# williamedwards/autompc

Hardware: AMD Instinct MI355X
Metric: MPC solves/sec (MPPI, n_samples x horizon rollouts + update per solve) (higher is better)
Workload: dtype f64; 1 GPU; c3: HalfCheetah (17-dim state, 6-dim ctrl), MLP 2x256, MPPI 4096 samples x 30 horizon; random-weight model, QuadCost Q=I R=0.01I F=I, sigma=1 lmda=1, 1 independent solve(s) per step per GPU, noise=device; n_samples=4096, horizon=30, state_dim=17, ctrl_dim=6, parallelism=independent solves per GPU (dp1)

## Files before the change

autompc_amd/csrc/mlp_tile.hpp:

```cpp
#pragma once
#include <hip/hip_runtime.h>

#include <type_traits>

#include "probe.hpp"

namespace ampc {

constexpr int kMaxHidden = 4;
constexpr int kMaxWaves = 8;

typedef double d4 __attribute__((ext_vector_type(4)));
typedef float f4 __attribute__((ext_vector_type(4)));

template <typename T> struct Acc;
template <> struct Acc<double> { using type = d4; };
template <> struct Acc<float> { using type = f4; };

__device__ __forceinline__ d4 mfma16(double a, double b, d4 c) {
  if constexpr (Probe::no_mfma) { c[0] += a * b; return c; }
  else return __builtin_amdgcn_mfma_f64_16x16x4f64(a, b, c, 0, 0, 0);
}
__device__ __forceinline__ f4 mfma16(float a, float b, f4 c) {
  if constexpr (Probe::no_mfma) { c[0] += a * b; return c; }
// ... 306 lines not shown
        b[nt] = __builtin_bit_cast(T, __builtin_amdgcn_raw_buffer_load_b64(r, vo + nt * 8u, sb, 0));
      else
        b[nt] = __builtin_bit_cast(T, __builtin_amdgcn_raw_buffer_load_b32(r, vo + nt * 4u, sb, 0));
    }
  }
}

template <typename T, int NT, int G>
__device__ __forceinline__ void load_group(rsrc_t r, unsigned so, unsigned lo, int g, T (&b)[G][NT]) {
#pragma unroll
  for (int kk = 0; kk < G; ++kk) load_frag<T, NT>(r, so + (unsigned)(g * G + kk) * 64u * NT, lo, b[kk]);
}

struct NoSide { __device__ __forceinline__ void operator()() const {} };
struct NoGroups {};

template <typename T, int NT, int MT, int KS, int G, bool PIPE = false, bool OWN = false, int SG = G,
          bool APERM = false, bool SWAP = false, typename Mid = NoSide, typename Groups = NoGroups,
          typename OwnFrag = NoGroups>
__device__ __forceinline__ void layer_mma_static(const T* __restrict__ A, int a_stride,
                                                 rsrc_t wr, unsigned wl, int lane,
                                                 const T (&first)[G][NT],
                                                 typename Acc<T>::type (&acc)[MT][NT], int rot = 0,
                                                 Mid&& mid = Mid(), Groups&& group_at = Groups(),
                                                 OwnFrag&& own_at = OwnFrag()) {
  static_assert(KS % G == 0 && G % SG == 0, "group sizes must divide the k extent");
  constexpr int NG = KS / G;
  constexpr int NS = KS / SG;
  constexpr int FS = G / SG;
  static_assert(!OWN || (NG & (NG - 1)) == 0, "rotated k order needs a power-of-two group count");
  const int i = lane & 15, q = lane >> 4;
  constexpr bool PINNED = !std::is_same<typename std::decay<Groups>::type, NoGroups>::value;
  constexpr bool REG0 = !std::is_same<typename std::decay<OwnFrag>::type, NoGroups>::value;
  static_assert(!REG0 || (OWN && MT == 1), "register fragments: the wave's own group of a 16-row tile");
  const T* arow = A + (APERM ? act_row<T>(i) : i) * a_stride + q;
  auto sub_group = [&](int g, int sub) {
    if constexpr (PINNED) return group_at(g) + 4 * SG * sub;
    else return (OWN ? arow + 4 * G * ((g + rot) & (NG - 1)) : arow + 4 * G * g) + 4 * SG * sub;
  };
  T b[2][SG][NT];
  if constexpr (FS == 1) {
#pragma unroll
    for (int kk = 0; kk < SG; ++kk)
#pragma unroll
      for (int nt = 0; nt < NT; ++nt) b[0][kk][nt] = first[kk][nt];
  }
#pragma unroll
  for (int sgi = 0; sgi < NS; ++sgi) {
    if (sgi + 1 >= FS && sgi + 1 < NS) load_group<T, NT, SG>(wr, wl, (unsigned)lane * NT, sgi + 1, b[(sgi + 1) & 1]);
    const int g = sgi / FS;
    const auto ag = sub_group(g, sgi % FS);
#pragma unroll
    for (int kk = 0; kk < SG; ++kk) {
      T a[MT];
#pragma unroll
      for (int mt = 0; mt < MT; ++mt) {
        if constexpr (REG0) a[mt] = sgi < FS ? own_at(sgi * SG + kk) : ag[4 * kk];
        else a[mt] = ag[mt * 16 * a_stride + 4 * kk];
      }
#pragma unroll
      for (int mt = 0; mt < MT; ++mt)
#pragma unroll
        for (int nt = 0; nt < NT; ++nt) {
          const T bv = (FS > 1 && sgi < FS) ? first[sgi * SG + kk][nt] : b[sgi & 1][kk][nt];
          constexpr bool REAL = KS < 16 ? kRealL0 : kRealHid;
          acc[mt][nt] = SWAP ? mfma16_x<REAL>(bv, a[mt], acc[mt][nt]) : mfma16_x<REAL>(a[mt], bv, acc[mt][nt]);
        }
    }
    if constexpr (PIPE && KS >= 8 && !Probe::no_sched) {
      if constexpr (Probe::vmem_first) {
        __builtin_amdgcn_sched_group_barrier(0x020, SG, 0);
        __builtin_amdgcn_sched_group_barrier(0x100, 2 * MT, 0);
#pragma unroll
        for (int i = 0; i < SG / 2; ++i) {
          __builtin_amdgcn_sched_group_barrier(0x008, 2 * MT * NT, 0);
          __builtin_amdgcn_sched_group_barrier(0x100, MT, 0);
        }
      } else if constexpr (sizeof(T) == 4 && (Probe::f32_ahead > 0 || Probe::f32_fine > 0)) {
        constexpr int AH = Probe::f32_ahead > 0 ? Probe::f32_ahead : 2;
        __builtin_amdgcn_sched_group_barrier(0x100, AH * MT, 0);
        if constexpr (Probe::f32_fine == 1) {
#pragma unroll
          for (int i = 0; i < SG; ++i) {
            __builtin_amdgcn_sched_group_barrier(0x008, MT * NT, 0);
            if (i + AH < SG) __builtin_amdgcn_sched_group_barrier(0x100, MT, 0);
            __builtin_amdgcn_sched_group_barrier(0x020, 1, 0);
          }
        } else if constexpr (Probe::f32_fine == 2) {
          constexpr int H1 = (MT * NT + 1) / 2, H2 = MT * NT - H1;
#pragma unroll
          for (int i = 0; i < SG; ++i) {
            __builtin_amdgcn_sched_group_barrier(0x008, H1, 0);
            if (i + AH < SG) __builtin_amdgcn_sched_group_barrier(0x100, MT, 0);
            if (H2 > 0) __builtin_amdgcn_sched_group_barrier(0x008, H2, 0);
            __builtin_amdgcn_sched_group_barrier(0x020, 1, 0);
          }
        } else if constexpr (Probe::f32_fine == 3) {
#pragma unroll
          for (int i = 0; i < SG; ++i) {
            __builtin_amdgcn_sched_group_barrier(0x008, MT * NT, 0);
            __builtin_amdgcn_sched_group_barrier(0x020, 1, 0);
            if (i + AH < SG) __builtin_amdgcn_sched_group_barrier(0x100, MT, 0);
          }
        } else {
#pragma unroll
          for (int i = 0; i < SG / 2; ++i) {
            __builtin_amdgcn_sched_group_barrier(0x008, 2 * MT * NT, 0);
            if (2 * i + AH < SG) __builtin_amdgcn_sched_group_barrier(0x100, MT, 0);
            if (2 * i + AH + 1 < SG) __builtin_amdgcn_sched_group_barrier(0x100, MT, 0);
            __builtin_amdgcn_sched_group_barrier(0x020, 2, 0);
          }
        }
      } else if (REG0 && sgi < FS) {
#pragma unroll
        for (int i = 0; i < SG / 2; ++i) {
          __builtin_amdgcn_sched_group_barrier(0x008, 2 * MT * NT, 0);
          __builtin_amdgcn_sched_group_barrier(0x020, 2, 0);
        }
      } else {
        __builtin_amdgcn_sched_group_barrier(0x100, 2 * MT, 0);
#pragma unroll
        for (int i = 0; i < SG / 2; ++i) {
          __builtin_amdgcn_sched_group_barrier(0x008, 2 * MT * NT, 0);
          __builtin_amdgcn_sched_group_barrier(0x100, MT, 0);
          __builtin_amdgcn_sched_group_barrier(0x020, 2, 0);
        }
      }
    }
    if (OWN && sgi == FS - 1) {
      lds_barrier();
      mid();
    }
    if constexpr (Probe::valu_pad) {
      if (KS >= 16 && sgi >= 2 && sgi < 10) {
        int padv = lane;
#pragma unroll
        for (int pi = 0; pi < 8; ++pi) asm volatile("v_add_u32 %0, %0, 1" : "+v"(padv));
        asm volatile("" :: "v"(padv));
      }
    }
    if constexpr (Probe::valu_pad64) {
      if (KS >= 16 && sgi >= 2 && sgi < 10) {
        double padd = (double)lane;
#pragma unroll
        for (int pi = 0; pi < 8; ++pi) asm volatile("v_add_f64 %0, %0, 1.0" : "+v"(padd));
        asm volatile("" :: "v"(padd));
      }
    }
  }
}


template <typename T, int NT, int MT, int W, bool DERIV = false, int LEAN = 0, typename SH = DynShape,
          bool WIDE = false, bool PINNED = false>
struct TileNet {
  using acc_t = typename Acc<T>::type;
  static constexpr int M = 16 * MT;
  static constexpr int HP = 16 * NT * W;
  static constexpr int KSH = HP / 4;
  static constexpr int KSW = KSH / W;
  static constexpr int KS0MAX = 12;
  static constexpr int GH = 8;
  static constexpr int NOMAX = WIDE ? 4 : 2;
  static constexpr bool OWN = (16 * NT == 4 * GH) && (((KSH / GH) & (KSH / GH - 1)) == 0);
  static constexpr bool PIN = PINNED && SH::kStatic && sizeof(T) == 8;
  static constexpr bool CHAIN = PIN && MT == 1 && !DERIV && !WIDE && LEAN == 0;
  static constexpr int BR = (CHAIN && W == 8) ? 4 : 1;
  static constexpr bool CHAIN_BIAS_LDS = CHAIN && BR == 1;

  static constexpr int KS0RES = sizeof(T) == 4 ? KS0MAX : 6;
  T pf0[KS0RES][NT];
  __device__ __forceinline__ static bool resident0(const MlpDev<T>& m) {
    return !Probe::no_res0 && LEAN < 2 && (sizeof(T) == 4 || MT == 1) && m.k1p <= 4 * KS0RES;
  }

  __device__ __forceinline__ static unsigned slice0(const MlpDev<T>& m, int w) {
    return (unsigned)(m.W(0) - m.WB()) + (unsigned)w * (unsigned)(m.k1p / 4) * 64u * NT;
  }
  __device__ __forceinline__ static unsigned slice_h(const MlpDev<T>& m, int l, int w) {
    return (unsigned)(m.W(l) - m.WB()) + (unsigned)w * (unsigned)KSH * 64u * NT;
  }
  rsrc_t wr;
  template <int KS> __device__ __forceinline__ const T (&first0() const)[KS][NT] {
    return reinterpret_cast<const T(&)[KS][NT]>(pf0);
  }
  template <int KS> __device__ __forceinline__ T (&first0())[KS][NT] {
    return reinterpret_cast<T(&)[KS][NT]>(pf0);
  }

  static constexpr bool RESIDENT_OUT = WIDE || (LEAN < 2 && !(MT == 4 && sizeof(T) == 8));
  T wout[KSW][NOMAX];

  __device__ __forceinline__ static void load_out(const MlpDev<T>& m, int w, int lane,
                                                  T (&dst)[KSW][NOMAX]) {
    if constexpr (WIDE) {
      const int tiles = m.nxp / 16;
      const T* wl = m.W(m.n_hidden) + ((size_t)w * KSW * 64 + lane) * tiles;
#pragma unroll
      for (int ks = 0; ks < KSW; ++ks)
#pragma unroll
        for (int n = 0; n < NOMAX; ++n) dst[ks][n] = n < tiles ? wl[(size_t)ks * 64 * tiles + n] : T(0);
    } else if (m.nxp == 16) {
      const T* wl = m.W(m.n_hidden) + ((size_t)w * KSW * 64 + lane);
#pragma unroll
      for (int ks = 0; ks < KSW; ++ks) { dst[ks][0] = wl[ks * 64]; dst[ks][1] = T(0); }
    } else {
      const T* wl = m.W(m.n_hidden) + ((size_t)w * KSW * 64 + lane) * 2;
#pragma unroll
      for (int ks = 0; ks < KSW; ++ks) { const vec_t<T, 2> v = *reinterpret_cast<const vec_t<T, 2>*>(wl + ks * 128); dst[ks][0] = v[0]; dst[ks][1] = v[1]; }
      if (m.tail4) {
        const T* wt = m.WT() + ((size_t)w * KSW * 64 + lane);
#pragma unroll
        for (int ks = 0; ks < KSW; ++ks) dst[ks][1] = wt[ks * 64];
      }
    }
  }

  static constexpr bool RESIDENT_BIAS = LEAN < 1 && (MT == 1);
  static constexpr int kResBias = 2;
  T bias_r[kResBias][NT][BR];
  T pfn[GH][NT];
  ProbeWave<Probe::wave_time> probe;

  lds_ptr<const T> bq_;
  static constexpr int RS = sizeof(T) == 8 ? 4 : 1;
  static constexpr int NGH = KSH / GH;
  lds_ptr<T> ep_[2][4];
  lds_ptr<const T> rd_[2][NGH];
  lds_ptr<const T> ro_;
  lds_ptr<const T> x0_;
  lds_ptr<T> pp_, pt_;
  int w_;

  __device__ __forceinline__ void pin(const MlpDev<T>& m_in, const TileLds& L_in, T* lds) {
    if constexpr (PIN) {
      const MlpDev<T> m = SH::template fold<T>(m_in);
      const TileLds L = SH::template fold_lds<T, M, W>(L_in);
      const int lane = threadIdx.x & 63;
      const int w = w_ = __builtin_amdgcn_readfirstlane(threadIdx.x >> 6);
      const int i = lane & 15, q = lane >> 4;
      const int as = L.act_stride;
      const bool pingpong = L.act2 != L.act;
#pragma unroll
      for (int b = 0; b < 2; ++b) {
        T* buf = lds + (b ? L.act2 : L.act);
        const bool read = b == 0 ? m.n_hidden > 1 : (pingpong && m.n_hidden > 2);
        const bool written = CHAIN ? read : (b == 0 || pingpong);
#pragma unroll
        for (int r = 0; r < 4; ++r) {
          if constexpr (CHAIN)
            ep_[b][r] = (written && r == 0) ? lds_pin(buf + i * as + 16 * NT * w + q) : lds_ptr<T>(nullptr);
          else
            ep_[b][r] = written ? lds_pin(buf + (act_row<T>(acc_row<T>(q, 0)) + RS * r) * as + 16 * NT * w + i) : ep_[0][r];
        }
#pragma unroll
        for (int g = 0; g < NGH; ++g) {
          const T* grp = buf + act_row<T>(i) * as + q + 4 * GH * (OWN ? ((g + w) & (NGH - 1)) : g);
          const bool used = OWN ? (g > 0 || !CHAIN) : g == 0;
          rd_[b][g] = (read && used) ? lds_pin(grp) : lds_ptr<const T>(nullptr);
        }
      }
      const T* last = lds + ((pingpong && ((m.n_hidden - 1) & 1)) ? L.act2 : L.act);
      ro_ = CHAIN ? lds_ptr<const T>(nullptr) : lds_pin(last + act_row<T>(i) * as + q + 4 * w * KSW);
      bq_ = (CHAIN && (CHAIN_BIAS_LDS || m.n_hidden > kResBias)) ? lds_pin(static_cast<const T*>(lds + L.bias + 16 * NT * w + q))
                                             : lds_ptr<const T>(nullptr);
      x0_ = lds_pin(static_cast<const T*>(lds + L.xu + i * L.xu_stride + q));
      const int ps = part_stride((int)sizeof(T), m.nxp);
      T* part = lds + L.part + w * M * ps;
      pp_ = lds_pin(part + acc_row<T>(q, 0) * ps + i);
      pt_ = m.tail4 ? lds_pin(part + tail_row(lane) * ps + 16 + tail_col(lane)) : pp_;
    }
  }

  __device__ __forceinline__ void init(const MlpDev<T>& m_in) {
    const MlpDev<T> m = SH::template fold<T>(m_in);
    const int lane = threadIdx.x & 63;
    const int w = __builtin_amdgcn_readfirstlane(threadIdx.x >> 6);
#pragma unroll
    for (int l = 0; l < kResBias; ++l)
#pragma unroll
      for (int nt = 0; nt < NT; ++nt)
#pragma unroll
        for (int r = 0; r < BR; ++r) {
          const int col = CHAIN ? 4 * r + (lane >> 4) : (lane & 15);
          bias_r[l][nt][r] = (RESIDENT_BIAS && !CHAIN_BIAS_LDS && l < m.n_hidden) ? m.B(l)[16 * (NT * w + nt) + col] : T(0);
        }
    wr = weight_rsrc(m.WB());
    if constexpr (RESIDENT_OUT) load_out(m, w, lane, wout);
    load0_all(m);
    if (m.n_hidden > 1) load_group<T, NT, GH>(wr, slice_h(m, 1, w), (unsigned)lane * NT, 0, pfn);
  }

  __device__ __forceinline__ void load0_all(const MlpDev<T>& m_in) {
    const MlpDev<T> m = SH::template fold<T>(m_in);
    const int lane = threadIdx.x & 63;
    const int w = __builtin_amdgcn_readfirstlane(threadIdx.x >> 6);
    const unsigned wl = slice0(m, w);
    const int ks0 = resident0(m) ? m.k1p / 4 : 2;
#pragma unroll
    for (int ks = 0; ks < KS0RES; ++ks) {
      T tmp[NT];
#pragma unroll
      for (int nt = 0; nt < NT; ++nt) tmp[nt] = T(0);
      if (ks < ks0) load_frag<T, NT>(wr, wl + (unsigned)ks * 64u * NT, (unsigned)lane * NT, tmp);
#pragma unroll
      for (int nt = 0; nt < NT; ++nt) pf0[ks][nt] = tmp[nt];
    }
  }

  template <int KS, typename AP>
  __device__ __forceinline__ void layer0_resident(AP arow, int a_stride, acc_t (&acc)[MT][NT]) const {
    static_assert(KS <= KS0RES, "layer 0 wider than the resident buffer");
#pragma unroll
    for (int ks = 0; ks < KS; ++ks) {
      T a[MT];
#pragma unroll
      for (int mt = 0; mt < MT; ++mt) a[mt] = arow[mt * 16 * a_stride + 4 * ks];
#pragma unroll
      for (int mt = 0; mt < MT; ++mt)
#pragma unroll
        for (int nt = 0; nt < NT; ++nt)
          acc[mt][nt] = CHAIN ? mfma16_x<kRealL0>(pf0[ks][nt], a[mt], acc[mt][nt])
                              : mfma16_x<kRealL0>(a[mt], pf0[ks][nt], acc[mt][nt]);
    }
  }

  __device__ __forceinline__ void prefetch0(const MlpDev<T>& m_in) {
    const MlpDev<T> m = SH::template fold<T>(m_in);
    if (resident0(m)) return;
    const int lane = threadIdx.x & 63;
    const int w = __builtin_amdgcn_readfirstlane(threadIdx.x >> 6);
    load_group<T, NT, 2>(wr, slice0(m, w), (unsigned)lane * NT, 0, first0<2>());
  }

  __device__ __forceinline__ void run(const MlpDev<T>& m, const TileLds& L, T* lds,
                                      T* __restrict__ dz = nullptr, size_t dz_layer_stride = 0) {
    run_side(m, L, lds, [] {}, dz, dz_layer_stride);
  }

  template <typename Side>
  __device__ __forceinline__ void run_side(const MlpDev<T>& m_in, const TileLds& L_in, T* lds, Side&& side,
                                           T* __restrict__ dz = nullptr, size_t dz_layer_stride = 0) {
    const MlpDev<T> m = SH::template fold<T>(m_in);
    const TileLds L = SH::template fold_lds<T, M, W>(L_in);
    const int lane = threadIdx.x & 63;
    int w;
    if constexpr (PIN) { w = w_; asm volatile("" : "+s"(w)); }
    else w = __builtin_amdgcn_readfirstlane(threadIdx.x >> 6);
    const int i = lane & 15, q = lane >> 4;
    AMPC_PROBE_LOCALS(probe);
    T* act = lds + L.act;
    T* act_other = lds + L.act2;
    const bool pingpong = L.act2 != L.act;
    int cur = 0;
    const int as = L.act_stride;
    const int no = m.nxp / 16;
    static_assert(WIDE || GH * NT == KSW * NOMAX, "prefetch buffer shapes must coincide");
    auto prefetch_next = [&](int l_next) {
      if (l_next < m.n_hidden) {
        load_group<T, NT, GH>(wr, slice_h(m, l_next, w), (unsigned)lane * NT, 0, pfn);
      } else if constexpr (!RESIDENT_OUT) {
        T* flat = &pfn[0][0];
        if (m.nxp == 16) {
          const T* wl = m.W(m.n_hidden) + ((size_t)w * KSW * 64 + lane);
#pragma unroll
          for (int ks = 0; ks < KSW; ++ks) { flat[2 * ks] = wl[ks * 64]; flat[2 * ks + 1] = T(0); }
        } else {
          const T* wl = m.W(m.n_hidden) + ((size_t)w * KSW * 64 + lane) * 2;
#pragma unroll
          for (int ks = 0; ks < KSW; ++ks) {
            T two[2];
            const vec_t<T, 2> v2 = *reinterpret_cast<const vec_t<T, 2>*>(wl + ks * 128);
            two[0] = v2[0]; two[1] = v2[1];
            flat[2 * ks] = two[0];
            flat[2 * ks + 1] = two[1];
          }
          if (m.tail4) {
            const T* wt = m.WT() + ((size_t)w * KSW * 64 + lane);
#pragma unroll
            for (int ks = 0; ks < KSW; ++ks) flat[2 * ks + 1] = wt[ks * 64];
          }
        }
      }
    };
    auto wo = [&](int ks, int n) -> T {
      if constexpr (RESIDENT_OUT) return wout[ks][n];
      else return (&pfn[0][0])[2 * ks + n];
    };
    auto epilogue_k = [&](int l, acc_t (&acc)[MT][NT], T* dst, int db, auto kind_tag) {
      constexpr int KIND = decltype(kind_tag)::value;
      const T* bias = lds + L.bias + l * m.hpad + 16 * NT * w + i;
      T* d0 = dst + act_row<T>(acc_row<T>(q, 0)) * as + 16 * NT * w + i;
      T* z0 = DERIV ? dz + (size_t)l * dz_layer_stride + (size_t)acc_row<T>(q, 0) * m.hpad + 16 * NT * w + i : nullptr;
      auto bias_of = [&](int nt) -> T {
        if (RESIDENT_BIAS && l < kResBias) return (l == 0) ? bias_r[0][nt][0] : bias_r[kResBias - 1][nt][0];
        return bias[16 * nt];
      };
      auto emit = [&](int mt, int nt, int r, T bc) {
        const int ro = 16 * mt + RS * r;
        const T z = acc[mt][nt][r] + bc;
        if constexpr (PIN) (db ? ep_[1][r] : ep_[0][r])[16 * mt * as + 16 * nt] = act_apply<T>(KIND, z);
        else d0[ro * as + 16 * nt] = act_apply<T>(KIND, z);
        if (DERIV) z0[(size_t)ro * m.hpad + 16 * nt] = act_deriv<T>(KIND, z);
      };
      if constexpr (PIN) {
        T bc[NT];
#pragma unroll
        for (int nt = 0; nt < NT; ++nt) bc[nt] = bias_of(nt);
#pragma unroll
        for (int mt = 0; mt < MT; ++mt)
#pragma unroll
          for (int r = 0; r < 4; ++r)
#pragma unroll
            for (int nt = 0; nt < NT; ++nt) emit(mt, nt, r, bc[nt]);
      } else {
#pragma unroll
        for (int mt = 0; mt < MT; ++mt)
#pragma unroll
          for (int nt = 0; nt < NT; ++nt) {
            const T bc = bias_of(nt);
#pragma unroll
            for (int r = 0; r < 4; ++r) emit(mt, nt, r, bc);
          }
      }
    };
    auto epilogue = [&](int l, acc_t (&acc)[MT][NT], T* dst, int db) {
      switch (m.act) {
        case 0: epilogue_k(l, acc, dst, db, std::integral_constant<int, 0>{}); break;
        case 1: epilogue_k(l, acc, dst, db, std::integral_constant<int, 1>{}); break;
        case 2: epilogue_k(l, acc, dst, db, std::integral_constant<int, 2>{}); break;
        case 4: epilogue_k(l, acc, dst, db, std::integral_constant<int, 4>{}); break;
        default: epilogue_k(l, acc, dst, db, std::integral_constant<int, 3>{}); break;
      }
    };
    T own[NT][4];
    auto chain_k = [&](int l, acc_t (&acc)[MT][NT], int db, bool store, auto kind_tag) {
      constexpr int KIND = decltype(kind_tag)::value;
#pragma unroll
      for (int nt = 0; nt < NT; ++nt)
#pragma unroll
        for (int r = 0; r < 4; ++r) {
          T bc;
          if (!CHAIN_BIAS_LDS && l < kResBias) bc = (l == 0) ? bias_r[0][nt][r % BR] : bias_r[kResBias - 1][nt][r % BR];
          else bc = bq_[l * HP + 16 * nt + 4 * r];
          const T v = act_apply<T>(KIND, acc[0][nt][r] + bc);
          own[nt][r] = v;
          if (store) (db ? ep_[1][0] : ep_[0][0])[16 * nt + 4 * r] = v;
        }
    };
    auto epilogue_chain = [&](int l, acc_t (&acc)[MT][NT], int db, bool store) {
      switch (m.act) {
        case 0: chain_k(l, acc, db, store, std::integral_constant<int, 0>{}); break;
        case 1: chain_k(l, acc, db, store, std::integral_constant<int, 1>{}); break;
        case 2: chain_k(l, acc, db, store, std::integral_constant<int, 2>{}); break;
        case 4: chain_k(l, acc, db, store, std::integral_constant<int, 4>{}); break;
        default: chain_k(l, acc, db, store, std::integral_constant<int, 3>{}); break;
      }
    };

    bool side_done = false;
    {
      acc_t acc[MT][NT];
#pragma unroll
      for (int mt = 0; mt < MT; ++mt)
#pragma unroll
        for (int nt = 0; nt < NT; ++nt) acc[mt][nt] = acc_t{0, 0, 0, 0};
      const unsigned wl = slice0(m, w);
      const T* A = lds + L.xu;
      if (m.n_hidden == 1) prefetch_next(1);
      if (resident0(m)) {
        const auto arow0 = [&] {
          if constexpr (PIN) return x0_;
          else return A + i * L.xu_stride + q;
        }();
        switch (m.k1p) {
          case 8: layer0_resident<2>(arow0, L.xu_stride, acc); break;
          case 16: layer0_resident<4>(arow0, L.xu_stride, acc); break;
          case 24: layer0_resident<6>(arow0, L.xu_stride, acc); break;
          default:
            if constexpr (KS0RES >= 12) {
              switch (m.k1p) {
                case 32: layer0_resident<8>(arow0, L.xu_stride, acc); break;
                case 40: layer0_resident<10>(arow0, L.xu_stride, acc); break;
                default: layer0_resident<12>(arow0, L.xu_stride, acc); break;
              }
            }
            break;
        }
      } else {
        auto layer0_streamed = [&](auto ks) {
          layer_mma_static<T, NT, MT, decltype(ks)::value, 2, false, false, 2, false, CHAIN>(
              A, L.xu_stride, wr, wl, lane, first0<2>(), acc);
        };
        switch (m.k1p) {
          case 8: layer0_streamed(std::integral_constant<int, 2>{}); break;
          case 16: layer0_streamed(std::integral_constant<int, 4>{}); break;
          case 24: layer0_streamed(std::integral_constant<int, 6>{}); break;
          case 32: layer0_streamed(std::integral_constant<int, 8>{}); break;
          case 40: layer0_streamed(std::integral_constant<int, 10>{}); break;
          case 48: layer0_streamed(std::integral_constant<int, 12>{}); break;
          default:
            if constexpr (WIDE) {
              switch (m.k1p) {
                case 56: layer0_streamed(std::integral_constant<int, 14>{}); break;
                case 64: layer0_streamed(std::integral_constant<int, 16>{}); break;
                case 72: layer0_streamed(std::integral_constant<int, 18>{}); break;
                default: layer0_streamed(std::integral_constant<int, 20>{}); break;
              }
            } else {
              layer0_streamed(std::integral_constant<int, 12>{});
            }
            break;
        }
      }
      AMPC_MARK(2);
      if constexpr (CHAIN) epilogue_chain(0, acc, 0, m.n_hidden > 1);
      else epilogue(0, acc, act, 0);
    }
    if (!OWN && m.n_hidden > 1) lds_barrier();
    AMPC_MARK(3);

    for (int l = 1; l < m.n_hidden; ++l) {
      acc_t acc[MT][NT];
#pragma unroll
      for (int mt = 0; mt < MT; ++mt)
#pragma unroll
        for (int nt = 0; nt < NT; ++nt) {
          acc[mt][nt] = acc_t{0, 0, 0, 0};
        }
      constexpr int SGH = (sizeof(T) == 8 && !Probe::sg8) ? GH / 2 : GH;
      auto mid = [&] {
        if (!Probe::side_late && l == 1) { side(); side_done = true; }
      };
      auto pinned_group = [&](int g) {
        if constexpr (OWN) return cur ? rd_[1][g] : rd_[0][g];
        else return (cur ? rd_[1][0] : rd_[0][0]) + 4 * GH * g;
      };
      if constexpr (CHAIN && OWN)
        layer_mma_static<T, NT, MT, KSH, GH, (W == 8), OWN, SGH, true, true>(
            act, as, wr, slice_h(m, l, w), lane, pfn, acc, w, mid, pinned_group,
            [&](int kk) { return own[kk >> 2][kk & 3]; });
      else if constexpr (PIN)
        layer_mma_static<T, NT, MT, KSH, GH, (W == 8), OWN, SGH, true, CHAIN>(
            act, as, wr, slice_h(m, l, w), lane, pfn, acc, w, mid, pinned_group);
      else
        layer_mma_static<T, NT, MT, KSH, GH, (W == 8), OWN, SGH, true>(
            act, as, wr, slice_h(m, l, w), lane, pfn, acc, w, mid);
      AMPC_MARK(4);
      prefetch_next(l + 1);
      const bool stores = !CHAIN || l + 1 < m.n_hidden;
      if (!pingpong && stores) lds_barrier();
      AMPC_MARK(5);
      if constexpr (CHAIN) epilogue_chain(l, acc, pingpong ? cur ^ 1 : 0, stores);
      else epilogue(l, acc, act_other, pingpong ? cur ^ 1 : 0);
      if (!OWN && l + 1 < m.n_hidden) lds_barrier();
      AMPC_MARK(6);
      { T* tmp = act; act = act_other; act_other = tmp; }
      if (pingpong) cur ^= 1;
    }

    acc_t oacc[MT][NOMAX];
    T tacc[MT];
#pragma unroll
    for (int mt = 0; mt < MT; ++mt) {
      tacc[mt] = T(0);
#pragma unroll
      for (int n = 0; n < NOMAX; ++n) oacc[mt][n] = acc_t{0, 0, 0, 0};
    }
    {
      const auto arow = [&] {
        if constexpr (PIN) return ro_;
        else return static_cast<const T*>(act) + act_row<T>(i) * as + q + 4 * w * KSW;
      }();
      auto afrag = [&](int mt, int ks) -> T {
        if constexpr (CHAIN) return own[ks >> 2][ks & 3];
        else return arow[mt * 16 * as + 4 * ks];
      };
      if constexpr (WIDE) {
#pragma unroll
        for (int ks = 0; ks < KSW; ++ks)
#pragma unroll
          for (int mt = 0; mt < MT; ++mt) {
            const T a = afrag(mt, ks);
#pragma unroll
            for (int n = 0; n < NOMAX; ++n)
              if (n < no) oacc[mt][n] = mfma16_x<kRealOut>(a, wo(ks, n), oacc[mt][n]);
          }
      } else if (no == 1) {
#pragma unroll
        for (int ks = 0; ks < KSW; ++ks)
#pragma unroll
          for (int mt = 0; mt < MT; ++mt)
            oacc[mt][0] = mfma16_x<kRealOut>(afrag(mt, ks), wo(ks, 0), oacc[mt][0]);
      } else if (m.tail4) {
#pragma unroll
        for (int ks = 0; ks < KSW; ++ks)
#pragma unroll
          for (int mt = 0; mt < MT; ++mt) {
// ... 141 lines not shown
```

autompc_amd/csrc/mppi_kernels.hpp:

```cpp
#pragma once
#include "mlp_tile.hpp"
#include <stdint.h>

namespace ampc {

constexpr int kWG = 256;
constexpr int kWaves = 4;

template <typename T> struct MppiProblem {
  int N, H;
  int tile0;
  int cost_idx;
  T lam_over_sigma;
  T neg_inv_lambda;
  T sqrt_sigma;
  long long eps_off;
  long long epso_off;
  long long cost_off;
  int a_off;
  unsigned noise_id;
  int model;
};

template <typename T> struct MppiArgs {
  MlpDev<T> mlp;
  TileLds lds;
  int lds_aseq, lds_cost;
  int obs_dim, cost_stride;
  int term_mode, max_h;
  int cost_diag;
  int cost_affine;
  int lds_eps;
  int lds_red;
  int write_eps_out;
  int eps_inline;
  unsigned long long eps_seed, eps_stream;
  int hnu_stride;
  const T* costs_par;
  const T* bounds;
  const MppiProblem<T>* probs;
  const int* tile_prob;
  const T* x0;
  const T* act_in;
  T* act_out;
  const T* eps;
  T* eps_out;
  T* costs;
  T* term_last;
  T* u_out;
  T* tile_stat;
  T* tile_part;
  int* tile_done;
  int fused_combine;
  int n_ind;
  const T* ind_tab;
  const long long* model_delta;
  const int* tile_order;
  unsigned long long* done_flag;
  unsigned long long done_seq;
};

template <typename T>
__device__ __forceinline__ void publish_u(const MppiArgs<T>& args, int p, int nu, int j, T value) {
  args.u_out[p * nu + j] = value;
  if (args.done_flag) {
    __threadfence_system();
    if (j == 0) __hip_atomic_store(args.done_flag + p, args.done_seq, __ATOMIC_RELEASE, __HIP_MEMORY_SCOPE_SYSTEM);
  }
}

template <typename T> __device__ __forceinline__ T block_min(T v, T* scratch);
template <typename T> __device__ __forceinline__ T block_sum(T v, T* scratch);
template <typename T> __device__ __forceinline__ T wave_sum(T v);


template <typename T> __device__ __forceinline__ void st_agent(T* p, T v) {
  __hip_atomic_store(p, v, __ATOMIC_RELAXED, __HIP_MEMORY_SCOPE_AGENT);
}
template <typename T> __device__ __forceinline__ T ld_agent(const T* p) {
  return __hip_atomic_load(const_cast<T*>(p), __ATOMIC_RELAXED, __HIP_MEMORY_SCOPE_AGENT);
}

template <typename T, int NTHR>
__device__ __forceinline__ void finish_update_if_last(const MppiArgs<T>& args, const MppiProblem<T>& pr, int p,
                                                      int tile_m, T* scratch) {
  __shared__ int ticket_s;
  const int tid = threadIdx.x, nu = args.mlp.nu, H = pr.H;
  const int tiles = (pr.N + tile_m - 1) / tile_m;
  asm volatile("s_waitcnt vmcnt(0)" ::: "memory");
  __syncthreads();
  if (tid == 0) ticket_s = __hip_atomic_fetch_add(&args.tile_done[p], 1, __ATOMIC_RELAXED, __HIP_MEMORY_SCOPE_AGENT);
  __syncthreads();
  if (ticket_s != tiles - 1) return;
  if (tid == 0) __hip_atomic_store(&args.tile_done[p], 0, __ATOMIC_RELAXED, __HIP_MEMORY_SCOPE_AGENT);
  const T* st = args.tile_stat + 2 * (size_t)pr.tile0;
  T* sc = scratch;
  T* ss = scratch + tiles;
  T* part = ss + tiles;
  for (int i = tid; i < tiles; i += NTHR) { sc[i] = ld_agent(st + 2 * i); ss[i] = ld_agent(st + 2 * i + 1); }
  __syncthreads();
  T vmin = T(INFINITY);
  for (int i = 0; i < tiles; ++i) vmin = sc[i] < vmin ? sc[i] : vmin;
  __syncthreads();
  for (int i = tid; i < tiles; i += NTHR)
    sc[i] = (sc[i] < T(INFINITY)) ? exp(pr.neg_inv_lambda * (sc[i] - vmin)) : T(0);
  __syncthreads();
  T ssum = T(0);
  for (int i = 0; i < tiles; ++i) ssum += sc[i] * ss[i];
  const T* tp = args.tile_part + (size_t)pr.tile0 * args.hnu_stride;
  const int E = H * nu;
  for (int e0 = 0; e0 < E; e0 += NTHR) {
    const int ne = (E - e0) < NTHR ? (E - e0) : NTHR;
    const int NG = NTHR / ne;
    const int g = tid / ne, e = e0 + tid - g * ne;
    T acc = T(0);
    if (g < NG)
      for (int i = g; i < tiles; i += NG) acc += sc[i] * ld_agent(tp + (size_t)i * args.hnu_stride + e);
    __syncthreads();
    if (g < NG) part[tid] = acc;
    __syncthreads();
    if (tid < ne) {
      T tot = T(0);
      for (int k = 0; k < NG; ++k) tot += part[k * ne + tid];
      const int ee = e0 + tid, t = ee / nu, j = ee - t * nu;
      const int ts = (t + 1 < H) ? t + 1 : H - 1;
      const T a_new = args.act_in[pr.a_off + ts * nu + j] + tot / ssum;
      args.act_out[pr.a_off + ee] = a_new;
      if (t == 0) publish_u(args, p, nu, j, a_new * args.bounds[2 * nu + j]);
    }
  }
}

template <typename T, int NT, int MT, int W, typename SH = DynShape, bool WIDE = false>
__global__ __launch_bounds__(64 * W) void mppi_rollout_kernel(const MppiArgs<T> args) {
  extern __shared__ __attribute__((aligned(16))) unsigned char smem_raw[];
  T* lds = reinterpret_cast<T*>(smem_raw);
  using Net = TileNet<T, NT, MT, W, false, 0, SH, WIDE, true>;
  constexpr int M = 16 * MT, NTHR = 64 * W;
  constexpr int TPS = NTHR / M;
  constexpr int EPT = (16 + TPS - 1) / TPS;
  constexpr bool EXT = !SH::kStatic;
  const int tile = args.tile_order ? __builtin_amdgcn_readfirstlane(args.tile_order[blockIdx.x]) : (int)blockIdx.x;
  const int p = args.tile_prob[tile];
  const MppiProblem<T> pr = args.probs[p];
  const MlpDev<T> mlp = plan_model<SH, T>(args.mlp, [&] { return model_delta_of(args.model_delta, pr.model); });
  const TileLds L = SH::template fold_lds<T, M, W>(args.lds);
  const int tid = threadIdx.x;
  const int nx = mlp.nx, nu = mlp.nu, no = SH::kStatic ? SH::no : args.obs_dim;
  const int xs_ = L.xu_stride;
  const bool diag = args.cost_diag != 0, affine = args.cost_affine != 0;
  const int cost_stride = SH::kStatic ? cost_block_stride(SH::no, SH::nu) : args.cost_stride;
  const int lds_cost = SH::kStatic ? L.extra : args.lds_cost;
  const int lds_aseq = SH::kStatic ? round_up(L.extra + cost_stride + 3 * SH::nu, 4) : args.lds_aseq;

  const int first = (tile - pr.tile0) * M;
  const int H = pr.H, N = pr.N;

  if (W == 8) {
    if (__builtin_amdgcn_readfirstlane(threadIdx.x >> 6) < 4) __builtin_amdgcn_s_setprio(2);
    else __builtin_amdgcn_s_setprio(0);
  }
  Net net;
  net.init(mlp);
  net.pin(mlp, L, lds);

  T* aseq = lds + lds_aseq;
  T* cpar = lds + lds_cost;
  const T* Qm = cpar;
  const T* Rm = Qm + no * no;
  const T* Fm = Rm + nu * nu;
  const T* goal = Fm + no * no;
  const T* lin = goal + no;
  const T* lint = lin + no;
  const T* blo = cpar + cost_stride;
  const T* bhi = blo + nu;
  const T* bsc = bhi + nu;
  T* xu = lds + L.xu;

  tile_load_constants<T, W>(mlp, L, lds, M);
  for (int i = tid; i < cost_stride; i += NTHR)
    cpar[i] = args.costs_par[(size_t)pr.cost_idx * cost_stride + i];
  for (int i = tid; i < 3 * nu; i += NTHR) cpar[cost_stride + i] = args.bounds[i];
  for (int i = tid; i < H * nu; i += NTHR) {
    const int t = i / nu, j = i - t * nu;
    const int ts = (t + 1 < H) ? t + 1 : H - 1;
    aseq[i] = args.act_in[pr.a_off + ts * nu + j];
  }

  const int m = tid / TPS, r = tid % TPS;
  const int n = first + m;
  const bool valid = n < N;
  const T* eps_row = args.eps + pr.eps_off + (size_t)(valid ? n : 0) * H * nu;
  T* epso = args.eps_out + pr.epso_off;

  T c_part = T(0), ca_part = T(0);
  T e_next[EPT];
#pragma unroll
  for (int e = 0; e < EPT; ++e) {
    const int j = r + e * TPS;
    e_next[e] = (valid && j < nu) ? eps_row[j] : T(0);
  }
  __syncthreads();
  for (int i = tid; i < M * nx; i += NTHR) {
    const int row = i / nx, col = i - row * nx;
    xu[row * xs_ + col] = args.x0[p * nx + col];
  }

  T lo_r[EPT], hi_r[EPT], sc_r[EPT], rd_r[EPT];
  const T* eps_nx = eps_row + nu + r;
  auto actions = [&](int t) {
#pragma unroll
    for (int e = 0; e < EPT; ++e) {
      const int j = r + e * TPS;
      if (j < nu) {
        const T a = aseq[t * nu + j];
        T A = e_next[e] + a;
        A = A < lo_r[e] ? lo_r[e] : A;
        A = A > hi_r[e] ? hi_r[e] : A;
        const T ec = A - a;
        if (valid && args.write_eps_out) epso[((size_t)t * N + n) * nu + j] = ec;
        if (args.lds_eps >= 0) lds[args.lds_eps + (t * M + m) * nu + j] = ec;
        ca_part += A * ec;
        const T u = A * sc_r[e];
        xu[m * xs_ + nx + j] = u;
        if (diag) c_part += rd_r[e] * u * u;
        if constexpr (Net::PIN) {
          if (t + 1 < H && valid) e_next[e] = eps_nx[e * TPS];
        } else {
          if (t + 1 < H) e_next[e] = valid ? eps_row[(t + 1) * nu + j] : T(0);
        }
      }
    }
    if constexpr (Net::PIN) eps_nx += nu;
  };
#pragma unroll
  for (int e = 0; e < EPT; ++e) {
    const int j = r + e * TPS;
    lo_r[e] = j < nu ? blo[j] : T(0);
    hi_r[e] = j < nu ? bhi[j] : T(0);
    sc_r[e] = j < nu ? bsc[j] : T(0);
    rd_r[e] = j < nu ? Rm[j * nu + j] : T(0);
  }
  actions(0);
  __syncthreads();
  if (diag) c_part += quad_rows<T>(Qm, xu + m * xs_, goal, no, r, TPS, true);
  if (affine) {
    if (diag) c_part += affine_rows<T>(lin, xu + m * xs_, goal, no, r, TPS, T(0));
    if (r == 0) c_part += T(H) * lint[no];
  }

  AMPC_PROBE_KERNEL_BEGIN(net.probe);
  constexpr int XPT = ((WIDE ? 64 : 32) + TPS - 1) / TPS;
  T qd_r[XPT], gl_r[XPT], ql_r[XPT];
#pragma unroll
  for (int e = 0; e < XPT; ++e) {
    const int i = r + e * TPS;
    qd_r[e] = (diag && i < no) ? Qm[i * no + i] : T(0);
    gl_r[e] = i < no ? goal[i] : T(0);
    ql_r[e] = (diag && i < no) ? lin[i] : T(0);
  }
  for (int t = 0; t < H; ++t) {
    AMPC_PROBE_STEP(net.probe, t == 5);
    AMPC_MARK(0);
    if constexpr (EXT)
      if (args.n_ind) c_part += indicator_rows<T>(args.ind_tab, args.n_ind, xu + m * xs_, 1, no, r, TPS);
    if (!diag && !Probe::no_cost) {
      c_part += quad_rows<T>(Qm, xu + m * xs_, goal, no, r, TPS, false);
      c_part += quad_rows<T>(Rm, xu + m * xs_ + nx, nullptr, nu, r, TPS, false);
      if (affine) c_part += affine_rows<T>(lin, xu + m * xs_, goal, no, r, TPS, T(0));
    }
    AMPC_MARK(1);
    net.run_side(mlp, L, lds, [&] { if (t + 1 < H) actions(t + 1); });
#pragma unroll
    for (int e = 0; e < XPT; ++e) {
      const int i = r + e * TPS;
      if (i < nx) {
        const T xn = xu[m * xs_ + i] + Net::output(mlp, L, lds, m, i);
        xu[m * xs_ + i] = xn;
        if (diag && i < no && t + 1 < H) {
          const T d = xn - gl_r[e];
          c_part += (qd_r[e] * d + ql_r[e]) * d;
        }
      }
    }
    AMPC_MARK(12);
    AMPC_MARK(10);
    lds_barrier();
    AMPC_MARK(11);
  }

  AMPC_PROBE_KERNEL_END();
  T term = quad_rows<T>(Fm, xu + m * xs_, goal, no, r, TPS, diag);
  if (affine) term += affine_rows<T>(lint, xu + m * xs_, goal, no, r, TPS, lint[no + 1]);
  T c = c_part + pr.lam_over_sigma * ca_part;
  if (args.term_mode == 1) c += term;
#pragma unroll
  for (int off = TPS / 2; off > 0; off >>= 1) {
    c += __shfl_xor(c, off);
    term += __shfl_xor(term, off);
  }
  if (r == 0 && valid) {
    args.costs[pr.cost_off + n] = c;
    if (n == N - 1) args.term_last[p] = term;
  }
  if (args.lds_eps < 0) return;

  T* cred = lds + args.lds_red;
  T* sred = cred + M;
  if (r == 0) cred[m] = valid ? c : T(INFINITY);
  __syncthreads();
  T mw = cred[0];
  for (int i = 1; i < M; ++i) mw = cred[i] < mw ? cred[i] : mw;
  const bool dead_tile = !(mw < T(INFINITY));
  if (tid < M)
    sred[tid] = (first + tid < N && !dead_tile) ? exp(pr.neg_inv_lambda * (cred[tid] - mw)) : T(0);
  __syncthreads();
  const T* el = lds + args.lds_eps;
  T* tp = args.tile_part + (size_t)tile * args.hnu_stride;
  for (int e = tid; e < H * nu; e += NTHR) {
    const int t = e / nu, j = e - t * nu;
    T s = T(0);
    for (int i = 0; i < M; ++i) s += sred[i] * el[(t * M + i) * nu + j];
    tp[e] = s;
  }
  if (tid == 0) {
    T ss = T(0);
    for (int i = 0; i < M; ++i) ss += sred[i];
    args.tile_stat[2 * tile] = mw;
    args.tile_stat[2 * tile + 1] = ss;
  }
}

constexpr int kMaxNu = 16;

template <typename T>
__device__ __forceinline__ void philox_normal_pair(T* __restrict__ out, long long count, T scale, uint64_t seed,
                                                   uint64_t stream, uint32_t id, long long pair);
template <typename T> struct NoiseAhead {
  T* eps;
  unsigned long long seed, stream;
};

template <typename T>
__global__ __launch_bounds__(kWG) void mppi_combine_kernel(const MppiArgs<T> args, int tile_m,
                                                           const NoiseAhead<T> ahead) {
  __shared__ T scratch[kWaves];
  __shared__ T red[kWaves][kMaxNu];
  const int p = blockIdx.y, t = blockIdx.x, tid = threadIdx.x;
  const MppiProblem<T> pr = args.probs[p];
  if (t >= args.max_h) {
    if (ahead.eps)
      philox_normal_pair<T>(ahead.eps + pr.eps_off, (long long)pr.N * pr.H * args.mlp.nu, pr.sqrt_sigma, ahead.seed,
                            ahead.stream, pr.noise_id, (long long)(t - args.max_h) * kWG + tid);
    return;
  }
  if (t >= pr.H) return;
  const int nu = args.mlp.nu, H = pr.H;
  const int tiles = (pr.N + tile_m - 1) / tile_m;
  const T* st = args.tile_stat + 2 * (size_t)pr.tile0;
  T vmin = st[0];
  for (int i = tid; i < tiles; i += kWG) vmin = st[2 * i] < vmin ? st[2 * i] : vmin;
  vmin = block_min(vmin, scratch);
  const T* tp = args.tile_part + (size_t)pr.tile0 * args.hnu_stride + t * nu;
  T ssum = T(0);
  T acc[kMaxNu];
#pragma unroll
  for (int j = 0; j < kMaxNu; ++j) acc[j] = T(0);
  for (int i = tid; i < tiles; i += kWG) {
    if (!(st[2 * i] < T(INFINITY))) continue;
    const T sc = exp(pr.neg_inv_lambda * (st[2 * i] - vmin));
    ssum += sc * st[2 * i + 1];
    const T* row = tp + (size_t)i * args.hnu_stride;
#pragma unroll
    for (int j = 0; j < kMaxNu; ++j)
      if (j < nu) acc[j] += sc * row[j];
  }
  ssum = block_sum(ssum, scratch);
#pragma unroll
  for (int j = 0; j < kMaxNu; ++j)
    if (j < nu) {
      const T s = wave_sum(acc[j]);
      if ((tid & 63) == 0) red[tid >> 6][j] = s;
    }
  __syncthreads();
  if (tid < nu) {
    T s = red[0][tid];
#pragma unroll
    for (int w = 1; w < kWaves; ++w) s += red[w][tid];
    const int ts = (t + 1 < H) ? t + 1 : H - 1;
    const T a_new = args.act_in[pr.a_off + ts * nu + tid] + s / ssum;
    args.act_out[pr.a_off + t * nu + tid] = a_new;
    if (t == 0) publish_u(args, p, nu, tid, a_new * args.bounds[2 * nu + tid]);
  }
}

template <typename T> __device__ __forceinline__ T wave_min(T v) {
#pragma unroll
  for (int off = 32; off > 0; off >>= 1) { T o = __shfl_xor(v, off); v = o < v ? o : v; }
  return v;
}
template <typename T> __device__ __forceinline__ T wave_sum(T v) {
#pragma unroll
  for (int off = 32; off > 0; off >>= 1) v += __shfl_xor(v, off);
  return v;
}
template <typename T> __device__ __forceinline__ T block_min(T v, T* scratch) {
  v = wave_min(v);
  __syncthreads();
  if ((threadIdx.x & 63) == 0) scratch[threadIdx.x >> 6] = v;
  __syncthreads();
  T o = scratch[0];
#pragma unroll
  for (int w = 1; w < kWaves; ++w) o = scratch[w] < o ? scratch[w] : o;
  return o;
}
template <typename T> __device__ __forceinline__ T block_sum(T v, T* scratch) {
  v = wave_sum(v);
  __syncthreads();
  if ((threadIdx.x & 63) == 0) scratch[threadIdx.x >> 6] = v;
  __syncthreads();
  T o = scratch[0];
#pragma unroll
  for (int w = 1; w < kWaves; ++w) o += scratch[w];
  return o;
}

constexpr int kUpdateMaxN = 8192;

template <typename T>
__global__ __launch_bounds__(kWG) void mppi_update_kernel(const MppiArgs<T> args, const NoiseAhead<T> ahead) {
  extern __shared__ __attribute__((aligned(16))) unsigned char upd_smem[];
  T* wts = reinterpret_cast<T*>(upd_smem);
  const int p = blockIdx.y, t = blockIdx.x;
  const MppiProblem<T> pr = args.probs[p];
  if (t >= args.max_h) {
    if (ahead.eps)
      philox_normal_pair<T>(ahead.eps + pr.eps_off, (long long)pr.N * pr.H * args.mlp.nu, pr.sqrt_sigma, ahead.seed,
                            ahead.stream, pr.noise_id, (long long)(t - args.max_h) * kWG + threadIdx.x);
    return;
  }
  if (t >= pr.H) return;
  const int N = pr.N, nu = args.mlp.nu, tid = threadIdx.x;
  const bool cached = N <= kUpdateMaxN;
  T* scratch = wts + (cached ? N : 0);
  T* part = scratch + kWaves;
  const T* c = args.costs + pr.cost_off;
  const int active = (kWG / nu) * nu;
  const T* e = args.eps_out + pr.epso_off + (size_t)t * N * nu;
  constexpr int U = 8;
  const int total = N * nu;
  T pre[U];
#pragma unroll
  for (int k = 0; k < U; ++k) {
    const int idx = tid + k * active;
    pre[k] = (tid < active && idx < total) ? e[idx] : T(0);
  }

  T vmin = c[0];
  for (int n = tid; n < N; n += kWG) vmin = c[n] < vmin ? c[n] : vmin;
  vmin = block_min(vmin, scratch);
  T ssum = T(0);
  for (int n = tid; n < N; n += kWG) {
    const T s = exp(pr.neg_inv_lambda * (c[n] - vmin));
    if (cached) wts[n] = s;
    ssum += s;
  }
  ssum = block_sum(ssum, scratch);

  T acc = T(0);
  if (tid < active) {
    int n = tid / nu;
    const int dn = active / nu;
    int i = tid;
#pragma unroll
    for (int k = 0; k < U; ++k) {
      if (i < total) {
        const T wgt = cached ? wts[n] : exp(pr.neg_inv_lambda * (c[n] - vmin));
        acc += wgt * pre[k];
        i += active; n += dn;
      }
    }
    for (; i + (U - 1) * active < total; i += U * active, n += U * dn) {
      T ev[U];
#pragma unroll
      for (int k = 0; k < U; ++k) ev[k] = e[i + k * active];
#pragma unroll
      for (int k = 0; k < U; ++k) {
        const int nn = n + k * dn;
        const T wgt = cached ? wts[nn] : exp(pr.neg_inv_lambda * (c[nn] - vmin));
        acc += wgt * ev[k];
      }
    }
    for (; i < total; i += active, n += dn) {
      const T wgt = cached ? wts[n] : exp(pr.neg_inv_lambda * (c[n] - vmin));
      acc += wgt * e[i];
    }
  }
  part[tid] = tid < active ? acc : T(0);
  __syncthreads();
  if (tid < nu) {
    T s = T(0);
    for (int i = tid; i < active; i += nu) s += part[i];
    const int ts = (t + 1 < pr.H) ? t + 1 : pr.H - 1;
    const T a_new = args.act_in[pr.a_off + ts * nu + tid] + s / ssum;
    args.act_out[pr.a_off + t * nu + tid] = a_new;
    if (t == 0) publish_u(args, p, nu, tid, a_new * args.bounds[2 * nu + tid]);
  }
}

template <typename T>
__global__ void mppi_finalize_costs_kernel(const MppiArgs<T> args) {
  const int p = blockIdx.y;
  const MppiProblem<T> pr = args.probs[p];
  const int n = blockIdx.x * blockDim.x + threadIdx.x;
  if (n < pr.N) args.costs[pr.cost_off + n] += args.term_last[p];
}

template <typename T>
__global__ void closed_loop_record_kernel(const T* __restrict__ x_next, const T* __restrict__ u,
                                          T* __restrict__ x0, T* __restrict__ traj_obs,
                                          T* __restrict__ traj_ctrls, int B, int nx, int nu, int T1,
                                          int step) {
  const int i = blockIdx.x * blockDim.x + threadIdx.x;
  if (i < B * nx) {
    const int p = i / nx, c = i - p * nx;
    const T v = x_next[i];
    x0[i] = v;
    traj_obs[((size_t)p * T1 + step + 1) * nx + c] = v;
  }
  if (i < B * nu) {
    const int p = i / nu, c = i - p * nu;
    traj_ctrls[((size_t)p * T1 + step) * nu + c] = u[i];
  }
}

template <typename T>
__global__ void state_lift_kernel(const T* __restrict__ sim, T* __restrict__ x0, const T* __restrict__ prog,
                                  int B, int snx, int no, int n_basis) {
  const int i = blockIdx.x * blockDim.x + threadIdx.x;
  if (i >= B * n_basis * no) return;
  const int b = i / (n_basis * no), e = i - b * n_basis * no, f = e / no, j = e - f * no;
  const T o = sim[(size_t)b * snx + j];
  const int kind = (int)prog[2 * f];
// ... 22 lines not shown
```

Measured before the change: 3462 solves/s.

## Fold layer-0 bias into padded K column and streamline combine reduction

In the rollout MLP, the layer-0 bias is now written into the unused last padded K slot of the resident layer-0 weight fragment, and the input rows get a constant 1 in that column. The first-layer MFMA therefore produces the biased result directly, and ReLU is applied with raw inline-asm v_max_f64 that carries hand-placed s_nop hazard padding. In the combine kernel, the first tile's stats and row loads plus the act_in load are issued before the min reduction. The separate block_sum for the weight sum is folded into the same shared-memory reduction as the per-control sums, removing one barrier round. The inline asm with manual nops is brittle and relies on correct hazard counts.

```diff
diff --git a/autompc_amd/csrc/mlp_tile.hpp b/autompc_amd/csrc/mlp_tile.hpp
--- a/autompc_amd/csrc/mlp_tile.hpp
+++ b/autompc_amd/csrc/mlp_tile.hpp
@@ -482,7 +482,7 @@
 
 
 template <typename T, int NT, int MT, int W, bool DERIV = false, int LEAN = 0, typename SH = DynShape,
-          bool WIDE = false, bool PINNED = false>
+          bool WIDE = false, bool PINNED = false, bool BIAS0K = false>
 struct TileNet {
   using acc_t = typename Acc<T>::type;
   static constexpr int M = 16 * MT;
@@ -497,6 +497,7 @@
   static constexpr bool CHAIN = PIN && MT == 1 && !DERIV && !WIDE && LEAN == 0;
   static constexpr int BR = (CHAIN && W == 8) ? 4 : 1;
   static constexpr bool CHAIN_BIAS_LDS = CHAIN && BR == 1;
+  static constexpr bool BIAS0_IN_K = BIAS0K && CHAIN && !Probe::no_res0 && SH::k1p <= 24 && SH::nx + SH::nu < SH::k1p;
 
   static constexpr int KS0RES = sizeof(T) == 4 ? KS0MAX : 6;
   T pf0[KS0RES][NT];
@@ -613,11 +614,20 @@
 #pragma unroll
         for (int r = 0; r < BR; ++r) {
           const int col = CHAIN ? 4 * r + (lane >> 4) : (lane & 15);
-          bias_r[l][nt][r] = (RESIDENT_BIAS && !CHAIN_BIAS_LDS && l < m.n_hidden) ? m.B(l)[16 * (NT * w + nt) + col] : T(0);
+          if (BIAS0_IN_K && l == 0) bias_r[l][nt][r] = T(0);
+          else bias_r[l][nt][r] = (RESIDENT_BIAS && !CHAIN_BIAS_LDS && l < m.n_hidden) ? m.B(l)[16 * (NT * w + nt) + col] : T(0);
         }
     wr = weight_rsrc(m.WB());
     if constexpr (RESIDENT_OUT) load_out(m, w, lane, wout);
     load0_all(m);
+    if constexpr (BIAS0_IN_K) {
+      constexpr int ksb = SH::k1p / 4 - 1;
+#pragma unroll
+      for (int nt = 0; nt < NT; ++nt) {
+        const T b = m.B(0)[16 * (NT * w + nt) + (lane & 15)];
+        pf0[ksb][nt] = (lane >> 4) == 3 ? b : pf0[ksb][nt];
+      }
+    }
     if (m.n_hidden > 1) load_group<T, NT, GH>(wr, slice_h(m, 1, w), (unsigned)lane * NT, 0, pfn);
   }
 
@@ -635,6 +645,25 @@
       if (ks < ks0) load_frag<T, NT>(wr, wl + (unsigned)ks * 64u * NT, (unsigned)lane * NT, tmp);
 #pragma unroll
       for (int nt = 0; nt < NT; ++nt) pf0[ks][nt] = tmp[nt];
+    }
+  }
+
+  __device__ __forceinline__ static void relu0_raw(const acc_t (&a)[NT], T (&v)[NT][4]) {
+    if constexpr (NT == 2) {
+      asm("s_nop 15\n\ts_nop 2\n\t"
+          "v_max_f64 %0, %8, 0\n\tv_max_f64 %1, %9, 0\n\tv_max_f64 %2, %10, 0\n\tv_max_f64 %3, %11, 0\n\t"
+          "v_max_f64 %4, %12, 0\n\tv_max_f64 %5, %13, 0\n\tv_max_f64 %6, %14, 0\n\tv_max_f64 %7, %15, 0\n\ts_nop 1"
+          : "=&v"(v[0][0]), "=&v"(v[0][1]), "=&v"(v[0][2]), "=&v"(v[0][3]), "=&v"(v[1][0]), "=&v"(v[1][1]),
+            "=&v"(v[1][2]), "=&v"(v[1][3])
+          : "v"(a[0][0]), "v"(a[0][1]), "v"(a[0][2]), "v"(a[0][3]), "v"(a[1][0]), "v"(a[1][1]), "v"(a[1][2]),
+            "v"(a[1][3]));
+    } else {
+#pragma unroll
+      for (int nt = 0; nt < NT; ++nt)
+        asm("s_nop 15\n\ts_nop 2\n\t"
+            "v_max_f64 %0, %4, 0\n\tv_max_f64 %1, %5, 0\n\tv_max_f64 %2, %6, 0\n\tv_max_f64 %3, %7, 0\n\ts_nop 1"
+            : "=&v"(v[nt][0]), "=&v"(v[nt][1]), "=&v"(v[nt][2]), "=&v"(v[nt][3])
+            : "v"(a[nt][0]), "v"(a[nt][1]), "v"(a[nt][2]), "v"(a[nt][3]));
     }
   }
 
@@ -766,14 +795,23 @@
     T own[NT][4];
     auto chain_k = [&](int l, acc_t (&acc)[MT][NT], int db, bool store, auto kind_tag) {
       constexpr int KIND = decltype(kind_tag)::value;
+      T raw0[NT][4];
+      if constexpr (BIAS0_IN_K && KIND == 0 && MT == 1)
+        if (l == 0) relu0_raw(acc[0], raw0);
 #pragma unroll
       for (int nt = 0; nt < NT; ++nt)
 #pragma unroll
         for (int r = 0; r < 4; ++r) {
-          T bc;
-          if (!CHAIN_BIAS_LDS && l < kResBias) bc = (l == 0) ? bias_r[0][nt][r % BR] : bias_r[kResBias - 1][nt][r % BR];
-          else bc = bq_[l * HP + 16 * nt + 4 * r];
-          const T v = act_apply<T>(KIND, acc[0][nt][r] + bc);
+          T v;
+          if (BIAS0_IN_K && l == 0) {
+            if constexpr (KIND == 0) v = raw0[nt][r];
+            else v = act_apply<T>(KIND, acc[0][nt][r]);
+          } else {
+            T bc;
+            if (!CHAIN_BIAS_LDS && l < kResBias) bc = (l == 0) ? bias_r[0][nt][r % BR] : bias_r[kResBias - 1][nt][r % BR];
+            else bc = bq_[l * HP + 16 * nt + 4 * r];
+            v = act_apply<T>(KIND, acc[0][nt][r] + bc);
+          }
           own[nt][r] = v;
           if (store) (db ? ep_[1][0] : ep_[0][0])[16 * nt + 4 * r] = v;
         }
diff --git a/autompc_amd/csrc/mppi_kernels.hpp b/autompc_amd/csrc/mppi_kernels.hpp
--- a/autompc_amd/csrc/mppi_kernels.hpp
+++ b/autompc_amd/csrc/mppi_kernels.hpp
@@ -135,7 +135,7 @@
 __global__ __launch_bounds__(64 * W) void mppi_rollout_kernel(const MppiArgs<T> args) {
   extern __shared__ __attribute__((aligned(16))) unsigned char smem_raw[];
   T* lds = reinterpret_cast<T*>(smem_raw);
-  using Net = TileNet<T, NT, MT, W, false, 0, SH, WIDE, true>;
+  using Net = TileNet<T, NT, MT, W, false, 0, SH, WIDE, true, true>;
   constexpr int M = 16 * MT, NTHR = 64 * W;
   constexpr int TPS = NTHR / M;
   constexpr int EPT = (16 + TPS - 1) / TPS;
@@ -205,6 +205,8 @@
     const int row = i / nx, col = i - row * nx;
     xu[row * xs_ + col] = args.x0[p * nx + col];
   }
+  if constexpr (Net::BIAS0_IN_K)
+    for (int i = tid; i < M; i += NTHR) xu[i * xs_ + SH::k1p - 1] = T(1);
 
   T lo_r[EPT], hi_r[EPT], sc_r[EPT], rd_r[EPT];
   const T* eps_nx = eps_row + nu + r;
@@ -345,7 +347,7 @@
 __global__ __launch_bounds__(kWG) void mppi_combine_kernel(const MppiArgs<T> args, int tile_m,
                                                            const NoiseAhead<T> ahead) {
   __shared__ T scratch[kWaves];
-  __shared__ T red[kWaves][kMaxNu];
+  __shared__ T red[kWaves][kMaxNu + 1];
   const int p = blockIdx.y, t = blockIdx.x, tid = threadIdx.x;
   const MppiProblem<T> pr = args.probs[p];
   if (t >= args.max_h) {
@@ -358,15 +360,31 @@
   const int nu = args.mlp.nu, H = pr.H;
   const int tiles = (pr.N + tile_m - 1) / tile_m;
   const T* st = args.tile_stat + 2 * (size_t)pr.tile0;
+  const T* tp = args.tile_part + (size_t)pr.tile0 * args.hnu_stride + t * nu;
+  const bool has0 = tid < tiles;
+  const int i0 = has0 ? tid : 0;
+  const T m0 = st[2 * i0], s0 = st[2 * i0 + 1];
+  T row0[kMaxNu];
+#pragma unroll
+  for (int j = 0; j < kMaxNu; ++j) row0[j] = j < nu ? tp[(size_t)i0 * args.hnu_stride + j] : T(0);
+  const int ts = (t + 1 < H) ? t + 1 : H - 1;
+  const T a_in = tid < nu ? args.act_in[pr.a_off + ts * nu + tid] : T(0);
   T vmin = st[0];
-  for (int i = tid; i < tiles; i += kWG) vmin = st[2 * i] < vmin ? st[2 * i] : vmin;
+  if (has0) vmin = m0 < vmin ? m0 : vmin;
+  for (int i = tid + kWG; i < tiles; i += kWG) vmin = st[2 * i] < vmin ? st[2 * i] : vmin;
   vmin = block_min(vmin, scratch);
-  const T* tp = args.tile_part + (size_t)pr.tile0 * args.hnu_stride + t * nu;
   T ssum = T(0);
   T acc[kMaxNu];
 #pragma unroll
   for (int j = 0; j < kMaxNu; ++j) acc[j] = T(0);
-  for (int i = tid; i < tiles; i += kWG) {
+  if (has0 && m0 < T(INFINITY)) {
+    const T sc = exp(pr.neg_inv_lambda * (m0 - vmin));
+    ssum += sc * s0;
+#pragma unroll
+    for (int j = 0; j < kMaxNu; ++j)
+      if (j < nu) acc[j] += sc * row0[j];
+  }
+  for (int i = tid + kWG; i < tiles; i += kWG) {
     if (!(st[2 * i] < T(INFINITY))) continue;
     const T sc = exp(pr.neg_inv_lambda * (st[2 * i] - vmin));
     ssum += sc * st[2 * i + 1];
@@ -375,20 +393,22 @@
     for (int j = 0; j < kMaxNu; ++j)
       if (j < nu) acc[j] += sc * row[j];
   }
-  ssum = block_sum(ssum, scratch);
 #pragma unroll
   for (int j = 0; j < kMaxNu; ++j)
     if (j < nu) {
       const T s = wave_sum(acc[j]);
       if ((tid & 63) == 0) red[tid >> 6][j] = s;
     }
+  {
+    const T s = wave_sum(ssum);
+    if ((tid & 63) == 0) red[tid >> 6][kMaxNu] = s;
+  }
   __syncthreads();
   if (tid < nu) {
-    T s = red[0][tid];
-#pragma unroll
-    for (int w = 1; w < kWaves; ++w) s += red[w][tid];
-    const int ts = (t + 1 < H) ? t + 1 : H - 1;
-    const T a_new = args.act_in[pr.a_off + ts * nu + tid] + s / ssum;
+    T s = red[0][tid], sw = red[0][kMaxNu];
+#pragma unroll
+    for (int w = 1; w < kWaves; ++w) { s += red[w][tid]; sw += red[w][kMaxNu]; }
+    const T a_new = a_in + s / sw;
     args.act_out[pr.a_off + t * nu + tid] = a_new;
     if (t == 0) publish_u(args, p, nu, tid, a_new * args.bounds[2 * nu + tid]);
   }
```

After: 3511 solves/s, median of 6. 1.01x the previous value.
